# cambrian-mllm/cambrian

Measured on NVIDIA H100. Metric: train_samples_per_sec, higher is better.
Workload: dtype bf16

## Files before the change

cambrian_b200/csrc/common.cuh:

```cuda
#pragma once
#include <cuda_runtime.h>
#include <cuda_bf16.h>
#include <cuda.h>
#include <stdint.h>
#include "wgmma.cuh"

namespace cb {

typedef __nv_bfloat16 bf16;

int set_error(int code, const char* fmt, ...);
#define CB_OK 0
#define CB_ERR_INVALID 1
#define CB_ERR_CUDA 2
#define CB_ERR_UNSUPPORTED 3

#define CB_CHECK_ARG(cond, ...)                                         \
  do {                                                                  \
    if (!(cond)) return cb::set_error(CB_ERR_INVALID, __VA_ARGS__);     \
  } while (0)

void count_launch();
#define CB_CUDA_LAUNCH_CHECK(name)                                                    \
  do {                                                                                \
    cb::count_launch();                                                               \
    cudaError_t _e = cudaGetLastError();                                              \
    if (_e != cudaSuccess)                                                            \
      return cb::set_error(CB_ERR_CUDA, "%s: %s", name, cudaGetErrorString(_e));      \
  } while (0)

int device_sm_count();

__device__ __forceinline__ float warp_sum(float v) {
#pragma unroll
  for (int o = 16; o > 0; o >>= 1) v += __shfl_xor_sync(0xffffffffu, v, o);
  return v;
}
__device__ __forceinline__ float warp_max(float v) {
#pragma unroll
  for (int o = 16; o > 0; o >>= 1) v = fmaxf(v, __shfl_xor_sync(0xffffffffu, v, o));
  return v;
}

__device__ __forceinline__ float fast_exp2(float x) {
  float y;
  asm("ex2.approx.ftz.f32 %0, %1;" : "=f"(y) : "f"(x));
  return y;
}
__device__ __forceinline__ float fast_rcp(float x) {
  float y;
  asm("rcp.approx.ftz.f32 %0, %1;" : "=f"(y) : "f"(x));
  return y;
}
__device__ __forceinline__ float erf_fast(float x) {
  const float ax = fabsf(x);
  const float t = __fdividef(1.0f, fmaf(0.3275911f, ax, 1.0f));
  float y = fmaf(t, 1.061405429f, -1.453152027f);
  y = fmaf(t, y, 1.421413741f);
  y = fmaf(t, y, -0.284496736f);
  y = fmaf(t, y, 0.254829592f);
  const float r = fmaf(-t * y, __expf(-ax * ax), 1.0f);
  return copysignf(r, x);
}
__device__ __forceinline__ float gelu_erf(float x) {
  const float ax = fabsf(x);
  const float t = fast_rcp(fmaf(0.3275911f * 0.70710678118654752440f, ax, 1.0f));
  float y = fmaf(t, 1.061405429f, -1.453152027f);
  y = fmaf(t, y, 1.421413741f);
  y = fmaf(t, y, -0.284496736f);
  y = fmaf(t, y, 0.254829592f);
  const float e = fast_exp2(x * x * -0.72134752044448170368f);
  const float r = fmaf(-(y * t), e, 1.0f);
  const float hx = 0.5f * x;
  return fmaf(fabsf(hx), r, hx);
}
__device__ __forceinline__ float gelu_erf_grad(float x) {
  const float cdf = 0.5f * (1.0f + erf_fast(x * 0.70710678118654752440f));
  const float pdf = 0.39894228040143267794f * __expf(-0.5f * x * x);
  return cdf + x * pdf;
}
__device__ __forceinline__ float gelu_tanh(float x) {
  const float u = 0.7978845608028654f * (x + 0.044715f * x * x * x);
  return 0.5f * x * (1.0f + tanhf(u));
}
__device__ __forceinline__ float gelu_tanh_fast(float x) {
  const float u = 0.7978845608028654f * (x + 0.044715f * x * x * x);
  const float t = 1.0f - 2.0f * fast_rcp(1.0f + fast_exp2(2.0f * 1.44269504088896340736f * u));
  return 0.5f * x * (1.0f + t);
}
__device__ __forceinline__ float quick_gelu(float x) { return x * fast_rcp(1.0f + fast_exp2(-1.702f * 1.44269504088896340736f * x)); }
__device__ __forceinline__ float silu(float x) { return x * fast_rcp(1.0f + fast_exp2(-1.44269504088896340736f * x)); }

struct alignas(16) bf16x8 {
  __nv_bfloat162 v[4];
};
__device__ __forceinline__ void unpack8(const uint4& u, float* f) {
  const __nv_bfloat162* p = reinterpret_cast<const __nv_bfloat162*>(&u);
#pragma unroll
  for (int i = 0; i < 4; ++i) {
    float2 t = __bfloat1622float2(p[i]);
    f[2 * i] = t.x;
    f[2 * i + 1] = t.y;
  }
}
__device__ __forceinline__ uint4 pack8(const float* f) {
  uint4 u;
  __nv_bfloat162* p = reinterpret_cast<__nv_bfloat162*>(&u);
#pragma unroll
  for (int i = 0; i < 4; ++i) p[i] = __floats2bfloat162_rn(f[2 * i], f[2 * i + 1]);
  return u;
}
__device__ __forceinline__ uint4 ldg_nc(const void* p) {
  uint4 r;
  asm volatile("ld.global.nc.L1::no_allocate.v4.u32 {%0,%1,%2,%3}, [%4];"
               : "=r"(r.x), "=r"(r.y), "=r"(r.z), "=r"(r.w)
               : "l"(p));
  return r;
}

__device__ __forceinline__ uint32_t smem_u32(const void* p) {
  return static_cast<uint32_t>(__cvta_generic_to_shared(p));
}
__device__ __forceinline__ void mbar_init(uint32_t bar, uint32_t count) {
  asm volatile("mbarrier.init.shared::cta.b64 [%0], %1;" ::"r"(bar), "r"(count));
}
__device__ __forceinline__ void mbar_fence_init() {
  asm volatile("fence.mbarrier_init.release.cluster;" ::: "memory");
}
__device__ __forceinline__ void mbar_arrive_expect_tx(uint32_t bar, uint32_t bytes) {
  asm volatile("mbarrier.arrive.expect_tx.shared::cta.b64 _, [%0], %1;" ::"r"(bar), "r"(bytes)
               : "memory");
}
__device__ __forceinline__ void mbar_arrive(uint32_t bar) {
  asm volatile("mbarrier.arrive.shared::cta.b64 _, [%0];" ::"r"(bar) : "memory");
}
__device__ __forceinline__ void mbar_wait(uint32_t bar, uint32_t parity) {
  uint32_t done;
  do {
    asm volatile(
        "{\n"
        ".reg .pred p;\n"
        "mbarrier.try_wait.parity.shared::cta.b64 p, [%1], %2;\n"
        "selp.u32 %0, 1, 0, p;\n"
        "}\n"
        : "=r"(done)
        : "r"(bar), "r"(parity)
        : "memory");
  } while (!done);
}
__device__ __forceinline__ void st_shared_b32(uint32_t addr, uint32_t v) {
  asm volatile("st.shared.b32 [%0], %1;" ::"r"(addr), "r"(v) : "memory");
}
__device__ __forceinline__ void fence_proxy_async_smem() {
  asm volatile("fence.proxy.async.shared::cta;" ::: "memory");
}

__device__ __forceinline__ void tma_prefetch_desc(const CUtensorMap* m) {
  asm volatile("prefetch.tensormap [%0];" ::"l"(m) : "memory");
}
__device__ __forceinline__ void tma_load_3d(uint32_t smem_dst, const CUtensorMap* m, uint32_t bar,
                                            int c0, int c1, int c2) {
  asm volatile(
      "cp.async.bulk.tensor.3d.shared::cluster.global.mbarrier::complete_tx::bytes "
      "[%0], [%1, {%3, %4, %5}], [%2];"
      :
      : "r"(smem_dst), "l"(m), "r"(bar), "r"(c0), "r"(c1), "r"(c2)
      : "memory");
}
__device__ __forceinline__ void tma_load_4d(uint32_t smem_dst, const CUtensorMap* m, uint32_t bar,
                                            int c0, int c1, int c2, int c3) {
  asm volatile(
      "cp.async.bulk.tensor.4d.shared::cluster.global.mbarrier::complete_tx::bytes "
      "[%0], [%1, {%3, %4, %5, %6}], [%2];"
      :
      : "r"(smem_dst), "l"(m), "r"(bar), "r"(c0), "r"(c1), "r"(c2), "r"(c3)
      : "memory");
}
__device__ __forceinline__ void tma_store_3d(const CUtensorMap* m, uint32_t smem_src, int c0, int c1, int c2) {
  asm volatile("cp.async.bulk.tensor.3d.global.shared::cta.bulk_group [%0, {%2, %3, %4}], [%1];"
               :
               : "l"(m), "r"(smem_src), "r"(c0), "r"(c1), "r"(c2)
               : "memory");
}
__device__ __forceinline__ void bulk_commit() { asm volatile("cp.async.bulk.commit_group;" ::: "memory"); }
template <int N>
__device__ __forceinline__ void bulk_wait_read() {
  asm volatile("cp.async.bulk.wait_group.read %0;" ::"n"(N) : "memory");
}
template <int N>
__device__ __forceinline__ void bulk_wait() {
  asm volatile("cp.async.bulk.wait_group %0;" ::"n"(N) : "memory");
}
template <int N>
__device__ __forceinline__ void setmaxnreg_dec() { asm volatile("setmaxnreg.dec.sync.aligned.u32 %0;" ::"n"(N)); }
template <int N>
__device__ __forceinline__ void setmaxnreg_inc() { asm volatile("setmaxnreg.inc.sync.aligned.u32 %0;" ::"n"(N)); }
__device__ __forceinline__ void named_bar_sync(int id, int threads) {
  asm volatile("bar.sync %0, %1;" ::"r"(id), "r"(threads) : "memory");
}

__device__ __forceinline__ void wgmma_fence() { asm volatile("wgmma.fence.sync.aligned;" ::: "memory"); }
__device__ __forceinline__ void wgmma_commit() { asm volatile("wgmma.commit_group.sync.aligned;" ::: "memory"); }
template <int N>
__device__ __forceinline__ void wgmma_wait() {
  asm volatile("wgmma.wait_group.sync.aligned %0;" ::"n"(N) : "memory");
}
template <int R>
__device__ __forceinline__ void reg_fence(float (&d)[R]) {
#pragma unroll
  for (int i = 0; i < R; ++i) asm volatile("" : "+f"(d[i])::"memory");
}

__device__ __forceinline__ uint64_t make_smem_desc_sw128(uint32_t saddr, uint32_t lbo_bytes,
                                                         uint32_t sbo_bytes) {
  uint64_t d = 0;
  d |= static_cast<uint64_t>((saddr & 0x3FFFFu) >> 4);
  d |= static_cast<uint64_t>((lbo_bytes >> 4) & 0x3FFFu) << 16;
  d |= static_cast<uint64_t>((sbo_bytes >> 4) & 0x3FFFu) << 32;
  d |= static_cast<uint64_t>(1) << 62;
  return d;
}

__device__ __forceinline__ uint32_t pack_bf16x2(float lo, float hi) {
  __nv_bfloat162 t = __floats2bfloat162_rn(lo, hi);
  return *reinterpret_cast<uint32_t*>(&t);
}

}
```

cambrian_b200/csrc/gemm.cu:

```cuda
#include "common.cuh"
#include <algorithm>
#include <cstring>
#include <cudaTypedefs.h>
#include <mutex>

namespace cb {

constexpr int BM = 128;
constexpr int BK = 64;
constexpr int GEMM_THREADS = 288;
constexpr int GROUP_M = 16;

struct GemmEpilogue {
  void* C;
  long long ldc, bsc;
  const bf16* bias;
  const bf16* colscale;
  const bf16* residual;
  long long ldr, bsr;
  float alpha;
  int out_fp32;
  int accumulate;
  int pair_ok;
  int tma_store;
};
constexpr int ACT_SWIGLU_PAIR = 5;

constexpr int STG_BYTES = 64 * 64 * 2;
constexpr int STAGING_BYTES = 2 * 2 * STG_BYTES;

template <int BN>
struct GemmCfg {
  static constexpr int A_BYTES = BM * BK * 2;
  static constexpr int B_BYTES = BN * BK * 2;
  static constexpr int STAGE_BYTES = A_BYTES + B_BYTES;
  static constexpr int STAGES = (BN == 256) ? 4 : (BN == 128 ? 6 : 8);
  static constexpr int SMEM_BYTES = STAGES * STAGE_BYTES + STAGING_BYTES + 1024  + 256 ;
  static_assert(SMEM_BYTES <= 232448, "exceeds the 227 KB of shared memory a CTA may use");
};

template <int ACT>
__device__ __forceinline__ float apply_act(float v) {
  if constexpr (ACT == 1) return gelu_erf(v);
  else if constexpr (ACT == 2) return gelu_tanh_fast(v);
  else if constexpr (ACT == 3) return quick_gelu(v);
  else if constexpr (ACT == 4) return silu(v);
  else return v;
}

__device__ __forceinline__ void tile_to_mn(int r, int m_blocks, int n_blocks, int& mb, int& nb) {
  const int tpg = GROUP_M * n_blocks;
  const int g = r / tpg;
  const int first = g * GROUP_M;
  const int gs = min(GROUP_M, m_blocks - first);
  const int w = r - g * tpg;
  mb = first + w % gs;
  nb = w / gs;
}

template <int BN, int ACT>
__device__ __forceinline__ void fuse_row(const GemmEpilogue& ep, long long c_off, long long r_off, int col0, int N,
                                         float* acc, int h) {
  constexpr int J = BN / 8;
#pragma unroll
  for (int j = 0; j < J; ++j) {
    acc[4 * j + 2 * h] *= ep.alpha;
    acc[4 * j + 2 * h + 1] *= ep.alpha;
  }
  if (ep.bias) {
#pragma unroll
    for (int j = 0; j < J; ++j) {
      const int col = col0 + 8 * j;
      if (col < N) {
        const float2 t = __bfloat1622float2(*reinterpret_cast<const __nv_bfloat162*>(ep.bias + col));
        acc[4 * j + 2 * h] += t.x;
        acc[4 * j + 2 * h + 1] += t.y;
      }
    }
  }
  if constexpr (ACT != 0) {
#pragma unroll
    for (int j = 0; j < J; ++j) {
      acc[4 * j + 2 * h] = apply_act<ACT>(acc[4 * j + 2 * h]);
      acc[4 * j + 2 * h + 1] = apply_act<ACT>(acc[4 * j + 2 * h + 1]);
    }
  }
  if (ep.colscale) {
#pragma unroll
    for (int j = 0; j < J; ++j) {
      const int col = col0 + 8 * j;
      if (col < N) {
        const float2 t = __bfloat1622float2(*reinterpret_cast<const __nv_bfloat162*>(ep.colscale + col));
        acc[4 * j + 2 * h] *= t.x;
        acc[4 * j + 2 * h + 1] *= t.y;
      }
    }
  }
  if (ep.residual) {
#pragma unroll
    for (int j = 0; j < J; ++j) {
      const int col = col0 + 8 * j;
      if (col < N) {
        const float2 t = __bfloat1622float2(*reinterpret_cast<const __nv_bfloat162*>(ep.residual + r_off + col));
        acc[4 * j + 2 * h] += t.x;
        acc[4 * j + 2 * h + 1] += t.y;
      }
    }
  }
  if (ep.accumulate && ep.out_fp32) {
    const float* cr = reinterpret_cast<const float*>(ep.C) + c_off;
#pragma unroll
    for (int j = 0; j < J; ++j) {
      const int col = col0 + 8 * j;
      if (col < N) {
        const float2 o = *reinterpret_cast<const float2*>(cr + col);
        acc[4 * j + 2 * h] += o.x;
        acc[4 * j + 2 * h + 1] += o.y;
      }
    }
  } else if (ep.accumulate) {
    const bf16* cr = reinterpret_cast<const bf16*>(ep.C) + c_off;
#pragma unroll
    for (int j = 0; j < J; ++j) {
      const int col = col0 + 8 * j;
      if (col < N) {
        const float2 o = __bfloat1622float2(*reinterpret_cast<const __nv_bfloat162*>(cr + col));
        acc[4 * j + 2 * h] += o.x;
        acc[4 * j + 2 * h + 1] += o.y;
      }
    }
  }
}

template <int BN>
__device__ __forceinline__ void store_row(const GemmEpilogue& ep, long long c_off, int col0, int N, const float* acc,
                                          int h) {
#pragma unroll
  for (int j = 0; j < BN / 8; ++j) {
    const int col = col0 + 8 * j;
    if (col >= N) continue;
    const float x = acc[4 * j + 2 * h], y = acc[4 * j + 2 * h + 1];
    if (ep.out_fp32) *reinterpret_cast<float2*>(reinterpret_cast<float*>(ep.C) + c_off + col) = make_float2(x, y);
    else *reinterpret_cast<__nv_bfloat162*>(reinterpret_cast<bf16*>(ep.C) + c_off + col) = __floats2bfloat162_rn(x, y);
  }
}

template <int ACT>
__device__ __forceinline__ void epilogue_elems(const GemmEpilogue& ep, long long c_off, long long r_off, int col, int N,
                                               float v0, float v1) {
  v0 *= ep.alpha;
  v1 *= ep.alpha;
#pragma unroll
  for (int e = 0; e < 2; ++e) {
    const int c = col + e;
    if (c >= N) break;
    float v = e ? v1 : v0;
    if (ep.bias) v += __bfloat162float(ep.bias[c]);
    v = apply_act<ACT>(v);
    if (ep.colscale) v *= __bfloat162float(ep.colscale[c]);
    if (ep.residual) v += __bfloat162float(ep.residual[r_off + c]);
    if (ep.out_fp32) {
      float* cp = reinterpret_cast<float*>(ep.C) + c_off + c;
      *cp = ep.accumulate ? *cp + v : v;
    } else {
      bf16* cp = reinterpret_cast<bf16*>(ep.C) + c_off + c;
      *cp = __float2bfloat16(ep.accumulate ? __bfloat162float(*cp) + v : v);
    }
  }
}

template <int BN, bool A_MN, bool B_MN, int ACT>
__global__ void __launch_bounds__(GEMM_THREADS, 1)
gemm_bf16_wgmma(const __grid_constant__ CUtensorMap tmA, const __grid_constant__ CUtensorMap tmB,
                const __grid_constant__ CUtensorMap tmC, const __grid_constant__ CUtensorMap tmAux, int M, int N, int K,
                int tiles, GemmEpilogue ep) {
  using Cfg = GemmCfg<BN>;
  constexpr int STAGES = Cfg::STAGES;
  constexpr bool SWIGLU = ACT == ACT_SWIGLU_PAIR;
  extern __shared__ uint8_t smem_raw[];
  const uint32_t smem_base = (smem_u32(smem_raw) + 1023u) & ~1023u;
  const uint32_t stg_base = smem_base + STAGES * Cfg::STAGE_BYTES;
  const uint32_t bar_base = stg_base + STAGING_BYTES;
  auto full_bar = [&](int s) { return bar_base + 8u * s; };
  auto empty_bar = [&](int s) { return bar_base + 8u * (STAGES + s); };

  const int warp = threadIdx.x >> 5;
  const int lane = threadIdx.x & 31;
  const int m_blocks = (M + BM - 1) / BM;
  const int n_blocks = SWIGLU ? (N / 2) / (BN / 2) : (N + BN - 1) / BN;
  const int tiles_per_batch = m_blocks * n_blocks;
  const int num_kb = (K + BK - 1) / BK;

  if (warp == 8 && lane == 0) {
    tma_prefetch_desc(&tmA);
    tma_prefetch_desc(&tmB);
    for (int s = 0; s < STAGES; ++s) {
      mbar_init(full_bar(s), 1);
      mbar_init(empty_bar(s), 2);
    }
    mbar_fence_init();
  }
  __syncthreads();

  if (warp == 8) {
    if (lane == 0) {
      int stage = 0;
      uint32_t phase = 0;
      for (int r = blockIdx.x; r < tiles; r += gridDim.x) {
        const int b = r / tiles_per_batch;
        int mb, nb;
        tile_to_mn(r - b * tiles_per_batch, m_blocks, n_blocks, mb, nb);
        const int m0 = mb * BM;
        for (int kb = 0; kb < num_kb; ++kb) {
          mbar_wait(empty_bar(stage), phase ^ 1u);
          const uint32_t sa = smem_base + stage * Cfg::STAGE_BYTES;
          const uint32_t sb = sa + Cfg::A_BYTES;
          mbar_arrive_expect_tx(full_bar(stage), Cfg::STAGE_BYTES);
          const int k0 = kb * BK;
          if (!A_MN) {
            tma_load_3d(sa, &tmA, full_bar(stage), k0, m0, b);
          } else {
#pragma unroll
            for (int i = 0; i < BM / 64; ++i)
              tma_load_3d(sa + i * (64 * BK * 2), &tmA, full_bar(stage), m0 + 64 * i, k0, b);
          }
          if (SWIGLU) {
            tma_load_3d(sb, &tmB, full_bar(stage), k0, nb * (BN / 2), 0);
            tma_load_3d(sb + (BN / 2) * BK * 2, &tmB, full_bar(stage), k0, N / 2 + nb * (BN / 2), 0);
          } else if (!B_MN) {
            tma_load_3d(sb, &tmB, full_bar(stage), k0, nb * BN, b);
          } else {
#pragma unroll
            for (int i = 0; i < BN / 64; ++i)
              tma_load_3d(sb + i * (64 * BK * 2), &tmB, full_bar(stage), nb * BN + 64 * i, k0, b);
          }
          if (++stage == STAGES) {
            stage = 0;
            phase ^= 1u;
          }
        }
      }
    }
    return;
  }

  const int wg = warp >> 2;
  const bool wg_leader = (threadIdx.x & 127) == 0;
  const int srow = (warp & 3) * 16 + (lane >> 2);
  const int cq = 2 * (lane & 3);
  const uint32_t stg = stg_base + wg * (2 * STG_BYTES);
  uint32_t q = 0;
  if (wg_leader && ep.tma_store) {
    tma_prefetch_desc(&tmC);
    if (SWIGLU) tma_prefetch_desc(&tmAux);
  }

  auto store_subtile = [&](const CUtensorMap* map, int x, int x_end, int y, int z, auto pair) {
    const uint32_t buf = stg + (q & 1u) * STG_BYTES;
#pragma unroll
    for (int h = 0; h < 2; ++h) {
      const int row = srow + 8 * h;
#pragma unroll
      for (int j = 0; j < 8; ++j) {
        const __nv_bfloat162 v = pair(j, h);
        st_shared_b32(buf + row * 128 + ((j ^ (row & 7)) << 4) + 2 * cq, *reinterpret_cast<const uint32_t*>(&v));
      }
    }
    fence_proxy_async_smem();
    if (wg_leader) bulk_wait_read<0>();
    named_bar_sync(1 + wg, 128);
    if (wg_leader && x < x_end && y < M) {
      tma_store_3d(map, buf, x, y, z);
      bulk_commit();
    }
    ++q;
  };

  float acc[BN / 2];
  int stage = 0;
  uint32_t phase = 0;
  for (int r = blockIdx.x; r < tiles; r += gridDim.x) {
    const int b = r / tiles_per_batch;
    int mb, nb;
    tile_to_mn(r - b * tiles_per_batch, m_blocks, n_blocks, mb, nb);
    const int m0 = mb * BM;
#pragma unroll
    for (int i = 0; i < BN / 2; ++i) acc[i] = 0.f;
    int prev_stage = -1;
    for (int kb = 0; kb < num_kb; ++kb) {
      mbar_wait(full_bar(stage), phase);
      const uint32_t sa = smem_base + stage * Cfg::STAGE_BYTES + wg * (64 * 128);
      const uint32_t sb = smem_base + stage * Cfg::STAGE_BYTES + Cfg::A_BYTES;
      reg_fence(acc);
      wgmma_fence();
#pragma unroll
      for (int k = 0; k < BK / 16; ++k) {
        const uint64_t adesc = A_MN ? make_smem_desc_sw128(sa + k * 2048, 64 * BK * 2, 1024)
                                    : make_smem_desc_sw128(sa + k * 32, 0, 1024);
        const uint64_t bdesc = B_MN ? make_smem_desc_sw128(sb + k * 2048, 64 * BK * 2, 1024)
                                    : make_smem_desc_sw128(sb + k * 32, 0, 1024);
        WgmmaSS<BN, A_MN ? 1 : 0, B_MN ? 1 : 0>::mma(acc, adesc, bdesc, 1u);
      }
      wgmma_commit();
      wgmma_wait<1>();
      reg_fence(acc);
      if (prev_stage >= 0 && wg_leader) mbar_arrive(empty_bar(prev_stage));
      prev_stage = stage;
      if (++stage == STAGES) {
        stage = 0;
        phase ^= 1u;
      }
    }
    wgmma_wait<0>();
    reg_fence(acc);
    if (wg_leader) mbar_arrive(empty_bar(prev_stage));

    const int y0 = m0 + wg * 64;
    if constexpr (SWIGLU) {
      constexpr int JH = BN / 16;
      const int F = N >> 1;
      const int f0 = nb * (BN / 2);
#pragma unroll
      for (int s = 0; s < BN / 128; ++s)
        store_subtile(&tmC, f0 + 64 * s, N, y0, 0, [&](int j, int h) {
          return __floats2bfloat162_rn(acc[4 * (8 * s + j) + 2 * h], acc[4 * (8 * s + j) + 2 * h + 1]);
        });
#pragma unroll
      for (int s = 0; s < BN / 128; ++s)
        store_subtile(&tmC, F + f0 + 64 * s, N, y0, 0, [&](int j, int h) {
          return __floats2bfloat162_rn(acc[4 * (JH + 8 * s + j) + 2 * h], acc[4 * (JH + 8 * s + j) + 2 * h + 1]);
        });
#pragma unroll
      for (int s = 0; s < BN / 128; ++s)
        store_subtile(&tmAux, f0 + 64 * s, F, y0, 0, [&](int j, int h) {
          const float2 g = __bfloat1622float2(
              __floats2bfloat162_rn(acc[4 * (8 * s + j) + 2 * h], acc[4 * (8 * s + j) + 2 * h + 1]));
          const float2 u = __bfloat1622float2(
              __floats2bfloat162_rn(acc[4 * (JH + 8 * s + j) + 2 * h], acc[4 * (JH + 8 * s + j) + 2 * h + 1]));
          return __floats2bfloat162_rn(silu(g.x) * u.x, silu(g.y) * u.y);
        });
    } else {
      const int n0 = nb * BN;
#pragma unroll
      for (int h = 0; h < 2; ++h) {
        const int row = y0 + srow + 8 * h;
        if (row >= M) continue;
        const long long c_off = static_cast<long long>(b) * ep.bsc + static_cast<long long>(row) * ep.ldc;
        const long long r_off = static_cast<long long>(b) * ep.bsr + static_cast<long long>(row) * ep.ldr;
        if (ep.pair_ok) {
          fuse_row<BN, ACT>(ep, c_off, r_off, n0 + cq, N, acc, h);
          if (!ep.tma_store) store_row<BN>(ep, c_off, n0 + cq, N, acc, h);
          continue;
        }
#pragma unroll
        for (int j = 0; j < BN / 8; ++j) {
          if (n0 + 8 * j >= N) break;
          epilogue_elems<ACT>(ep, c_off, r_off, n0 + 8 * j + cq, N, acc[4 * j + 2 * h], acc[4 * j + 2 * h + 1]);
        }
      }
      if (ep.tma_store) {
#pragma unroll
        for (int s = 0; s < BN / 64; ++s)
          store_subtile(&tmC, n0 + 64 * s, N, y0, b, [&](int j, int h) {
            return __floats2bfloat162_rn(acc[4 * (8 * s + j) + 2 * h], acc[4 * (8 * s + j) + 2 * h + 1]);
          });
      }
    }
  }
  if (wg_leader) bulk_wait<0>();
}

static PFN_cuTensorMapEncodeTiled_v12000 get_encode_fn() {
  static PFN_cuTensorMapEncodeTiled_v12000 fn = nullptr;
  static std::once_flag once;
  std::call_once(once, [] {
    void* p = nullptr;
    cudaDriverEntryPointQueryResult q;
    if (cudaGetDriverEntryPoint("cuTensorMapEncodeTiled", &p, cudaEnableDefault, &q) == cudaSuccess &&
        q == cudaDriverEntryPointSuccess)
      fn = reinterpret_cast<PFN_cuTensorMapEncodeTiled_v12000>(p);
  });
  return fn;
}

int make_tmap_bf16_3d(CUtensorMap* out, const void* base, uint64_t inner, uint64_t rows, uint64_t batch,
                      uint64_t ld_elems, uint64_t batch_stride_elems, uint32_t box_rows) {
  auto fn = get_encode_fn();
  if (!fn) return set_error(CB_ERR_CUDA, "cuTensorMapEncodeTiled entry point not available");
  if ((reinterpret_cast<uintptr_t>(base) & 15u) != 0)
    return set_error(CB_ERR_INVALID, "TMA operand base must be 16-byte aligned");
  if ((ld_elems % 8) != 0 || (batch > 1 && (batch_stride_elems % 8) != 0))
    return set_error(CB_ERR_INVALID, "TMA operand strides must be multiples of 8 elements (ld=%llu)",
                     (unsigned long long)ld_elems);
  cuuint64_t dims[3] = {inner, rows, batch};
  cuuint64_t bs = (batch > 1) ? batch_stride_elems * 2 : ld_elems * 2 * (rows ? rows : 1);
  cuuint64_t strides[2] = {ld_elems * 2, bs};
  cuuint32_t box[3] = {64, box_rows, 1};
  cuuint32_t estr[3] = {1, 1, 1};
  CUresult r = fn(out, CU_TENSOR_MAP_DATA_TYPE_BFLOAT16, 3, const_cast<void*>(base), dims, strides, box,
                  estr, CU_TENSOR_MAP_INTERLEAVE_NONE, CU_TENSOR_MAP_SWIZZLE_128B,
                  CU_TENSOR_MAP_L2_PROMOTION_L2_256B, CU_TENSOR_MAP_FLOAT_OOB_FILL_NONE);
  if (r == CUDA_ERROR_INVALID_CONTEXT) {
    cudaFree(0);
    r = fn(out, CU_TENSOR_MAP_DATA_TYPE_BFLOAT16, 3, const_cast<void*>(base), dims, strides, box, estr,
           CU_TENSOR_MAP_INTERLEAVE_NONE, CU_TENSOR_MAP_SWIZZLE_128B, CU_TENSOR_MAP_L2_PROMOTION_L2_256B,
           CU_TENSOR_MAP_FLOAT_OOB_FILL_NONE);
  }
  if (r != CUDA_SUCCESS) return set_error(CB_ERR_CUDA, "cuTensorMapEncodeTiled failed (%d)", (int)r);
  return CB_OK;
}

struct GemmMaps {
  CUtensorMap a, b, c, aux;
};

template <int BN, bool A_MN, bool B_MN, int ACT>
static int launch_gemm(const GemmMaps& tm, int M, int N, int K, int batch, const GemmEpilogue& ep,
                       cudaStream_t stream) {
  using Cfg = GemmCfg<BN>;
  auto kern = gemm_bf16_wgmma<BN, A_MN, B_MN, ACT>;
  static bool attr_set = false;
  if (!attr_set) {
    cudaError_t e = cudaFuncSetAttribute(kern, cudaFuncAttributeMaxDynamicSharedMemorySize, Cfg::SMEM_BYTES);
    if (e != cudaSuccess) return set_error(CB_ERR_CUDA, "gemm smem attr: %s", cudaGetErrorString(e));
    attr_set = true;
  }
  const int n_blocks = (ACT == ACT_SWIGLU_PAIR) ? (N / 2) / (BN / 2) : (N + BN - 1) / BN;
  const long long tiles = (long long)((M + BM - 1) / BM) * n_blocks * batch;
  CB_CHECK_ARG(tiles < (1LL << 31), "gemm: %lld tiles exceed the grid", tiles);
  const unsigned grid = (unsigned)std::min<long long>(tiles, device_sm_count());
  kern<<<grid, GEMM_THREADS, Cfg::SMEM_BYTES, stream>>>(tm.a, tm.b, tm.c, tm.aux, M, N, K, (int)tiles, ep);
  CB_CUDA_LAUNCH_CHECK("gemm_bf16_wgmma");
  return CB_OK;
}

template <int BN>
static int dispatch_major(int a_mn, int b_mn, int act, const GemmMaps& tm, int M, int N, int K, int batch,
                          const GemmEpilogue& ep, cudaStream_t stream) {
  if (!a_mn && !b_mn) {
    switch (act) {
      case 1: return launch_gemm<BN, false, false, 1>(tm, M, N, K, batch, ep, stream);
      case 2: return launch_gemm<BN, false, false, 2>(tm, M, N, K, batch, ep, stream);
      case 3: return launch_gemm<BN, false, false, 3>(tm, M, N, K, batch, ep, stream);
      case 4: return launch_gemm<BN, false, false, 4>(tm, M, N, K, batch, ep, stream);
      default: return launch_gemm<BN, false, false, 0>(tm, M, N, K, batch, ep, stream);
    }
  }
  if (!a_mn && b_mn) return launch_gemm<BN, false, true, 0>(tm, M, N, K, batch, ep, stream);
  if (a_mn && !b_mn) return launch_gemm<BN, true, false, 0>(tm, M, N, K, batch, ep, stream);
  return launch_gemm<BN, true, true, 0>(tm, M, N, K, batch, ep, stream);
}

int gemm_bf16(const void* A, const void* B, void* C, int M, int N, int K, int batch, long long lda,
              long long ldb, long long ldc, long long bsa, long long bsb, long long bsc, int a_mn, int b_mn,
              const void* bias, const void* colscale, const void* residual, long long ldr, long long bsr,
              float alpha, int act, int out_fp32, int accumulate, int force_bn, cudaStream_t stream) {
  CB_CHECK_ARG(M > 0 && N > 0 && K > 0 && batch > 0, "gemm: empty problem M=%d N=%d K=%d batch=%d", M, N, K,
               batch);
  CB_CHECK_ARG(A && B && C, "gemm: null operand");
  CB_CHECK_ARG(act >= 0 && act <= 4, "gemm: unknown activation %d", act);
  CB_CHECK_ARG(act == 0 || (!a_mn && !b_mn), "gemm: a fused activation needs K-major operands (forward layout)");
  CB_CHECK_ARG(force_bn == 0 || force_bn == 64 || force_bn == 128 || force_bn == 256, "gemm: bad BLOCK_N %d", force_bn);
  int bn = force_bn;
  if (bn == 0) {
    const int sms = device_sm_count();
    const long long mb = (M + BM - 1) / BM;
    auto tiles = [&](int b_n) { return mb * ((N + b_n - 1) / b_n) * batch; };
    if (N > 128 && tiles(256) >= (long long)(sms * 7) / 10) bn = 256;
    else if (N > 64 && tiles(128) >= (long long)(sms * 6) / 10) bn = 128;
    else if (N > 128 && tiles(64) > 2LL * sms) bn = 128;
    else bn = 64;
  }
  GemmMaps tm;
  std::memset(&tm, 0, sizeof(tm));
  int rc;
  if (!a_mn) rc = make_tmap_bf16_3d(&tm.a, A, K, M, batch, lda, bsa, BM);
  else       rc = make_tmap_bf16_3d(&tm.a, A, M, K, batch, lda, bsa, BK);
  if (rc) return rc;
  if (!b_mn) rc = make_tmap_bf16_3d(&tm.b, B, K, N, batch, ldb, bsb, bn);
  else       rc = make_tmap_bf16_3d(&tm.b, B, N, K, batch, ldb, bsb, BK);
  if (rc) return rc;
  GemmEpilogue ep;
  ep.C = C; ep.ldc = ldc; ep.bsc = bsc;
  ep.bias = static_cast<const bf16*>(bias);
  ep.colscale = static_cast<const bf16*>(colscale);
  ep.residual = static_cast<const bf16*>(residual);
  ep.ldr = ldr; ep.bsr = bsr;
  ep.alpha = alpha; ep.out_fp32 = out_fp32; ep.accumulate = accumulate;
  const unsigned calign = out_fp32 ? 7u : 3u;
  bool pair = (N % 2 == 0) && (ldc % 2 == 0) && (bsc % 2 == 0) && ((reinterpret_cast<uintptr_t>(C) & calign) == 0);
  if (residual)
    pair = pair && (ldr % 2 == 0) && (bsr % 2 == 0) && ((reinterpret_cast<uintptr_t>(residual) & 3u) == 0);
  if (bias) pair = pair && ((reinterpret_cast<uintptr_t>(bias) & 3u) == 0);
  if (colscale) pair = pair && ((reinterpret_cast<uintptr_t>(colscale) & 3u) == 0);
  ep.pair_ok = pair ? 1 : 0;
  const bool tma = pair && !out_fp32 && ((reinterpret_cast<uintptr_t>(C) & 15u) == 0) && ldc % 8 == 0 &&
                   (batch == 1 || (bsc > 0 && bsc % 8 == 0));
  if (tma && (rc = make_tmap_bf16_3d(&tm.c, C, N, M, batch, ldc, bsc, 64))) return rc;
  ep.tma_store = tma ? 1 : 0;
  switch (bn) {
    case 256: return dispatch_major<256>(a_mn, b_mn, act, tm, M, N, K, batch, ep, stream);
    case 128: return dispatch_major<128>(a_mn, b_mn, act, tm, M, N, K, batch, ep, stream);
    default:  return dispatch_major<64>(a_mn, b_mn, act, tm, M, N, K, batch, ep, stream);
  }
}

int gemm_swiglu_bf16(const void* A, const void* W, void* gu_out, void* act_out, int M, int F, int K, long long lda,
                     long long ldw, long long ld_gu, long long ld_act, cudaStream_t stream) {
  CB_CHECK_ARG(M > 0 && F > 0 && K > 0, "gemm_swiglu: empty problem M=%d F=%d K=%d", M, F, K);
  CB_CHECK_ARG(A && W && gu_out && act_out, "gemm_swiglu: null operand");
  CB_CHECK_ARG(F % 128 == 0, "gemm_swiglu: F=%d must be a multiple of 128 (whole 128-feature tiles, 16-byte aligned halves)", F);
  CB_CHECK_ARG(ld_gu % 8 == 0 && ld_act % 8 == 0 && ((reinterpret_cast<uintptr_t>(gu_out) & 15u) == 0) &&
                   ((reinterpret_cast<uintptr_t>(act_out) & 15u) == 0),
               "gemm_swiglu: outputs must be 16-byte aligned with ld %% 8 == 0");
  const int N = 2 * F;
  constexpr int BN = 256;
  GemmMaps tm;
  int rc;
  if ((rc = make_tmap_bf16_3d(&tm.a, A, K, M, 1, lda, 0, BM))) return rc;
  if ((rc = make_tmap_bf16_3d(&tm.b, W, K, N, 1, ldw, 0, BN / 2))) return rc;
  if ((rc = make_tmap_bf16_3d(&tm.c, gu_out, N, M, 1, ld_gu, 0, 64))) return rc;
  if ((rc = make_tmap_bf16_3d(&tm.aux, act_out, F, M, 1, ld_act, 0, 64))) return rc;
  GemmEpilogue ep;
  ep.C = gu_out; ep.ldc = ld_gu; ep.bsc = 0;
  ep.bias = nullptr; ep.colscale = nullptr; ep.residual = nullptr; ep.ldr = 0; ep.bsr = 0;
  ep.alpha = 1.0f; ep.out_fp32 = 0; ep.accumulate = 0; ep.pair_ok = 1; ep.tma_store = 1;
  return launch_gemm<BN, false, false, ACT_SWIGLU_PAIR>(tm, M, N, K, 1, ep, stream);
}

}
```

Before: 7.732.

## Prefetch GEMM epilogue residual/accumulate operand via TMA into pipeline ring stages

For GEMMs with a residual add or in-place accumulate and no activation, the producer warp now TMA-loads the residual (or existing C) tile into free smem ring stages after the K-loop loads. The consumer waits on those stages and adds the operand from shared memory during the TMA-store epilogue, instead of doing per-thread global loads in fuse_row. The stages are released at the start of the next tile. This targets uncoalesced epilogue global reads, but it occupies pipeline stages and adds synchronization complexity.

```diff
diff --git a/cambrian_b200/csrc/common.cuh b/cambrian_b200/csrc/common.cuh
--- a/cambrian_b200/csrc/common.cuh
+++ b/cambrian_b200/csrc/common.cuh
@@ -151,6 +151,11 @@
 __device__ __forceinline__ void st_shared_b32(uint32_t addr, uint32_t v) {
   asm volatile("st.shared.b32 [%0], %1;" ::"r"(addr), "r"(v) : "memory");
 }
+__device__ __forceinline__ uint32_t ld_shared_b32(uint32_t addr) {
+  uint32_t v;
+  asm volatile("ld.shared.b32 %0, [%1];" : "=r"(v) : "r"(addr) : "memory");
+  return v;
+}
 __device__ __forceinline__ void fence_proxy_async_smem() {
   asm volatile("fence.proxy.async.shared::cta;" ::: "memory");
 }
diff --git a/cambrian_b200/csrc/gemm.cu b/cambrian_b200/csrc/gemm.cu
--- a/cambrian_b200/csrc/gemm.cu
+++ b/cambrian_b200/csrc/gemm.cu
@@ -23,6 +23,7 @@
   int accumulate;
   int pair_ok;
   int tma_store;
+  int tma_operand;
 };
 constexpr int ACT_SWIGLU_PAIR = 5;
 
@@ -36,6 +37,10 @@
   static constexpr int STAGE_BYTES = A_BYTES + B_BYTES;
   static constexpr int STAGES = (BN == 256) ? 4 : (BN == 128 ? 6 : 8);
   static constexpr int SMEM_BYTES = STAGES * STAGE_BYTES + STAGING_BYTES + 1024  + 256 ;
+  static constexpr int OP_BOXES = 2 * (BN / 64);
+  static constexpr int BOXES_PER_STAGE = STAGE_BYTES / STG_BYTES;
+  static constexpr int OP_STAGES = (OP_BOXES + BOXES_PER_STAGE - 1) / BOXES_PER_STAGE;
+  static_assert(STAGE_BYTES % STG_BYTES == 0 && OP_STAGES < STAGES, "operand boxes must tile the ring stages");
   static_assert(SMEM_BYTES <= 232448, "exceeds the 227 KB of shared memory a CTA may use");
 };
 
@@ -58,7 +63,7 @@
   nb = w / gs;
 }
 
-template <int BN, int ACT>
+template <int BN, int ACT, bool OPS>
 __device__ __forceinline__ void fuse_row(const GemmEpilogue& ep, long long c_off, long long r_off, int col0, int N,
                                          float* acc, int h) {
   constexpr int J = BN / 8;
@@ -96,6 +101,7 @@
       }
     }
   }
+  if constexpr (OPS) return;
   if (ep.residual) {
 #pragma unroll
     for (int j = 0; j < J; ++j) {
@@ -169,7 +175,7 @@
   }
 }
 
-template <int BN, bool A_MN, bool B_MN, int ACT>
+template <int BN, bool A_MN, bool B_MN, int ACT, bool OPS>
 __global__ void __launch_bounds__(GEMM_THREADS, 1)
 gemm_bf16_wgmma(const __grid_constant__ CUtensorMap tmA, const __grid_constant__ CUtensorMap tmB,
                 const __grid_constant__ CUtensorMap tmC, const __grid_constant__ CUtensorMap tmAux, int M, int N, int K,
@@ -194,6 +200,7 @@
   if (warp == 8 && lane == 0) {
     tma_prefetch_desc(&tmA);
     tma_prefetch_desc(&tmB);
+    if (OPS) tma_prefetch_desc(ep.residual ? &tmAux : &tmC);
     for (int s = 0; s < STAGES; ++s) {
       mbar_init(full_bar(s), 1);
       mbar_init(empty_bar(s), 2);
@@ -239,6 +246,28 @@
             phase ^= 1u;
           }
         }
+        if (OPS) {
+          const CUtensorMap* op = ep.residual ? &tmAux : &tmC;
+          constexpr int S = BN / 64;
+          for (int t = 0; t < Cfg::OP_STAGES; ++t) {
+            mbar_wait(empty_bar(stage), phase ^ 1u);
+            const uint32_t base = smem_base + stage * Cfg::STAGE_BYTES;
+            const int i0 = t * Cfg::BOXES_PER_STAGE;
+            const int i1 = min(Cfg::OP_BOXES, i0 + Cfg::BOXES_PER_STAGE);
+            uint32_t bytes = 0;
+            for (int i = i0; i < i1; ++i)
+              if (nb * BN + 64 * (i % S) < N && m0 + 64 * (i / S) < M) bytes += STG_BYTES;
+            mbar_arrive_expect_tx(full_bar(stage), bytes);
+            for (int i = i0; i < i1; ++i) {
+              const int x = nb * BN + 64 * (i % S), y = m0 + 64 * (i / S);
+              if (x < N && y < M) tma_load_3d(base + (i - i0) * STG_BYTES, op, full_bar(stage), x, y, b);
+            }
+            if (++stage == STAGES) {
+              stage = 0;
+              phase ^= 1u;
+            }
+          }
+        }
       }
     }
     return;
@@ -255,30 +284,32 @@
     if (SWIGLU) tma_prefetch_desc(&tmAux);
   }
 
-  auto store_subtile = [&](const CUtensorMap* map, int x, int x_end, int y, int z, auto pair) {
-    const uint32_t buf = stg + (q & 1u) * STG_BYTES;
+  auto store_subtile = [&](const CUtensorMap* map, int x, int x_end, int y, int z, uint32_t op, auto pair) {
+    const uint32_t buf = op ? op : stg + (q & 1u) * STG_BYTES;
 #pragma unroll
     for (int h = 0; h < 2; ++h) {
       const int row = srow + 8 * h;
 #pragma unroll
       for (int j = 0; j < 8; ++j) {
-        const __nv_bfloat162 v = pair(j, h);
-        st_shared_b32(buf + row * 128 + ((j ^ (row & 7)) << 4) + 2 * cq, *reinterpret_cast<const uint32_t*>(&v));
+        const uint32_t addr = buf + row * 128 + ((j ^ (row & 7)) << 4) + 2 * cq;
+        const __nv_bfloat162 v = pair(j, h, addr);
+        st_shared_b32(addr, *reinterpret_cast<const uint32_t*>(&v));
       }
     }
     fence_proxy_async_smem();
-    if (wg_leader) bulk_wait_read<0>();
+    if (wg_leader && !op) bulk_wait_read<0>();
     named_bar_sync(1 + wg, 128);
     if (wg_leader && x < x_end && y < M) {
       tma_store_3d(map, buf, x, y, z);
       bulk_commit();
     }
-    ++q;
+    if (!op) ++q;
   };
 
   float acc[BN / 2];
   int stage = 0;
   uint32_t phase = 0;
+  int release_stage = -1;
   for (int r = blockIdx.x; r < tiles; r += gridDim.x) {
     const int b = r / tiles_per_batch;
     int mb, nb;
@@ -286,6 +317,13 @@
     const int m0 = mb * BM;
 #pragma unroll
     for (int i = 0; i < BN / 2; ++i) acc[i] = 0.f;
+    if (OPS && release_stage >= 0) {
+      if (wg_leader) {
+        bulk_wait_read<0>();
+        for (int t = 0; t < Cfg::OP_STAGES; ++t) mbar_arrive(empty_bar((release_stage + t) % STAGES));
+      }
+      release_stage = -1;
+    }
     int prev_stage = -1;
     for (int kb = 0; kb < num_kb; ++kb) {
       mbar_wait(full_bar(stage), phase);
@@ -322,17 +360,17 @@
       const int f0 = nb * (BN / 2);
 #pragma unroll
       for (int s = 0; s < BN / 128; ++s)
-        store_subtile(&tmC, f0 + 64 * s, N, y0, 0, [&](int j, int h) {
+        store_subtile(&tmC, f0 + 64 * s, N, y0, 0, 0u, [&](int j, int h, uint32_t) {
           return __floats2bfloat162_rn(acc[4 * (8 * s + j) + 2 * h], acc[4 * (8 * s + j) + 2 * h + 1]);
         });
 #pragma unroll
       for (int s = 0; s < BN / 128; ++s)
-        store_subtile(&tmC, F + f0 + 64 * s, N, y0, 0, [&](int j, int h) {
+        store_subtile(&tmC, F + f0 + 64 * s, N, y0, 0, 0u, [&](int j, int h, uint32_t) {
           return __floats2bfloat162_rn(acc[4 * (JH + 8 * s + j) + 2 * h], acc[4 * (JH + 8 * s + j) + 2 * h + 1]);
         });
 #pragma unroll
       for (int s = 0; s < BN / 128; ++s)
-        store_subtile(&tmAux, f0 + 64 * s, F, y0, 0, [&](int j, int h) {
+        store_subtile(&tmAux, f0 + 64 * s, F, y0, 0, 0u, [&](int j, int h, uint32_t) {
           const float2 g = __bfloat1622float2(
               __floats2bfloat162_rn(acc[4 * (8 * s + j) + 2 * h], acc[4 * (8 * s + j) + 2 * h + 1]));
           const float2 u = __bfloat1622float2(
@@ -348,7 +386,7 @@
         const long long c_off = static_cast<long long>(b) * ep.bsc + static_cast<long long>(row) * ep.ldc;
         const long long r_off = static_cast<long long>(b) * ep.bsr + static_cast<long long>(row) * ep.ldr;
         if (ep.pair_ok) {
-          fuse_row<BN, ACT>(ep, c_off, r_off, n0 + cq, N, acc, h);
+          fuse_row<BN, ACT, OPS>(ep, c_off, r_off, n0 + cq, N, acc, h);
           if (!ep.tma_store) store_row<BN>(ep, c_off, n0 + cq, N, acc, h);
           continue;
         }
@@ -359,11 +397,35 @@
         }
       }
       if (ep.tma_store) {
-#pragma unroll
-        for (int s = 0; s < BN / 64; ++s)
-          store_subtile(&tmC, n0 + 64 * s, N, y0, b, [&](int j, int h) {
-            return __floats2bfloat162_rn(acc[4 * (8 * s + j) + 2 * h], acc[4 * (8 * s + j) + 2 * h + 1]);
+        const int op_stage = stage;
+        if (OPS) {
+          for (int t = 0; t < Cfg::OP_STAGES; ++t) {
+            mbar_wait(full_bar(stage), phase);
+            if (++stage == STAGES) {
+              stage = 0;
+              phase ^= 1u;
+            }
+          }
+          release_stage = op_stage;
+        }
+#pragma unroll
+        for (int s = 0; s < BN / 64; ++s) {
+          const int i = wg * (BN / 64) + s;
+          const uint32_t op = OPS ? smem_base +
+                                                   ((op_stage + i / Cfg::BOXES_PER_STAGE) % STAGES) * Cfg::STAGE_BYTES +
+                                                   (i % Cfg::BOXES_PER_STAGE) * STG_BYTES
+                                             : 0u;
+          store_subtile(&tmC, n0 + 64 * s, N, y0, b, op, [&](int j, int h, uint32_t addr) {
+            float x = acc[4 * (8 * s + j) + 2 * h], y = acc[4 * (8 * s + j) + 2 * h + 1];
+            if (op) {
+              const uint32_t raw = ld_shared_b32(addr);
+              const float2 o = __bfloat1622float2(*reinterpret_cast<const __nv_bfloat162*>(&raw));
+              x += o.x;
+              y += o.y;
+            }
+            return __floats2bfloat162_rn(x, y);
           });
+        }
       }
     }
   }
@@ -414,11 +476,11 @@
   CUtensorMap a, b, c, aux;
 };
 
-template <int BN, bool A_MN, bool B_MN, int ACT>
+template <int BN, bool A_MN, bool B_MN, int ACT, bool OPS = false>
 static int launch_gemm(const GemmMaps& tm, int M, int N, int K, int batch, const GemmEpilogue& ep,
                        cudaStream_t stream) {
   using Cfg = GemmCfg<BN>;
-  auto kern = gemm_bf16_wgmma<BN, A_MN, B_MN, ACT>;
+  auto kern = gemm_bf16_wgmma<BN, A_MN, B_MN, ACT, OPS>;
   static bool attr_set = false;
   if (!attr_set) {
     cudaError_t e = cudaFuncSetAttribute(kern, cudaFuncAttributeMaxDynamicSharedMemorySize, Cfg::SMEM_BYTES);
@@ -437,6 +499,12 @@
 template <int BN>
 static int dispatch_major(int a_mn, int b_mn, int act, const GemmMaps& tm, int M, int N, int K, int batch,
                           const GemmEpilogue& ep, cudaStream_t stream) {
+  if (ep.tma_operand) {
+    if (!a_mn && !b_mn) return launch_gemm<BN, false, false, 0, true>(tm, M, N, K, batch, ep, stream);
+    if (!a_mn && b_mn) return launch_gemm<BN, false, true, 0, true>(tm, M, N, K, batch, ep, stream);
+    if (a_mn && !b_mn) return launch_gemm<BN, true, false, 0, true>(tm, M, N, K, batch, ep, stream);
+    return launch_gemm<BN, true, true, 0, true>(tm, M, N, K, batch, ep, stream);
+  }
   if (!a_mn && !b_mn) {
     switch (act) {
       case 1: return launch_gemm<BN, false, false, 1>(tm, M, N, K, batch, ep, stream);
@@ -498,6 +566,11 @@
                    (batch == 1 || (bsc > 0 && bsc % 8 == 0));
   if (tma && (rc = make_tmap_bf16_3d(&tm.c, C, N, M, batch, ldc, bsc, 64))) return rc;
   ep.tma_store = tma ? 1 : 0;
+  const bool res_tma = residual && ((reinterpret_cast<uintptr_t>(residual) & 15u) == 0) && ldr % 8 == 0 &&
+                       (batch == 1 || (bsr > 0 && bsr % 8 == 0));
+  const bool op_tma = tma && act == 0 && (residual ? res_tma && !accumulate : accumulate != 0);
+  if (op_tma && residual && (rc = make_tmap_bf16_3d(&tm.aux, residual, N, M, batch, ldr, bsr, 64))) return rc;
+  ep.tma_operand = op_tma ? 1 : 0;
   switch (bn) {
     case 256: return dispatch_major<256>(a_mn, b_mn, act, tm, M, N, K, batch, ep, stream);
     case 128: return dispatch_major<128>(a_mn, b_mn, act, tm, M, N, K, batch, ep, stream);
@@ -524,7 +597,7 @@
   GemmEpilogue ep;
   ep.C = gu_out; ep.ldc = ld_gu; ep.bsc = 0;
   ep.bias = nullptr; ep.colscale = nullptr; ep.residual = nullptr; ep.ldr = 0; ep.bsr = 0;
-  ep.alpha = 1.0f; ep.out_fp32 = 0; ep.accumulate = 0; ep.pair_ok = 1; ep.tma_store = 1;
+  ep.alpha = 1.0f; ep.out_fp32 = 0; ep.accumulate = 0; ep.pair_ok = 1; ep.tma_store = 1; ep.tma_operand = 0;
   return launch_gemm<BN, false, false, ACT_SWIGLU_PAIR>(tm, M, N, K, 1, ep, stream);
 }
 
```

New measurement: 7.820 (median of 6 runs). 1.01x the previous value.
